# KentaYoshii/Raymarcher

Hardware: AMD Instinct MI355X
Metric: Mpixels/s at 3840x2160 Mandelbulb, 256 march steps (higher is better)
Workload: dtype f32

## Files before the change

### raymarcher_amd/csrc/rm_device.hip.h

```cpp
#pragma once
#include "../../include/raymarcher_amd.h"
#include <type_traits>

#include "rm_math.hip.h"
#include "rm_internal.h"

namespace rm {

struct V3 { float x, y, z; };
struct V4 { float x, y, z, w; };

RM_DEV V3 v3(float x, float y, float z) { return V3{x, y, z}; }
RM_DEV V4 v4(float x, float y, float z, float w) { return V4{x, y, z, w}; }
RM_DEV V3 add(V3 a, V3 b) { return v3(a.x + b.x, a.y + b.y, a.z + b.z); }
RM_DEV V3 sub(V3 a, V3 b) { return v3(a.x - b.x, a.y - b.y, a.z - b.z); }
RM_DEV V3 mul(V3 a, V3 b) { return v3(a.x * b.x, a.y * b.y, a.z * b.z); }
RM_DEV V3 scale(V3 a, float s) { return v3(a.x * s, a.y * s, a.z * s); }
RM_DEV V3 neg(V3 a) { return v3(-a.x, -a.y, -a.z); }
RM_DEV V3 madd(V3 a, float s, V3 b) { return v3(fma(a.x, s, b.x), fma(a.y, s, b.y), fma(a.z, s, b.z)); }
RM_DEV float dot2(float ax, float ay, float bx, float by) { return fma(ay, by, ax * bx); }
RM_DEV float dot(V3 a, V3 b) { return fma(a.z, b.z, fma(a.y, b.y, a.x * b.x)); }
RM_DEV float len2(float x, float y) { return sqrt_(dot2(x, y, x, y)); }
RM_DEV float len(V3 a) { return sqrt_(dot(a, a)); }
RM_DEV V3 normalize(V3 a) { float inv = rcp_(len(a)); return scale(a, inv); }
// ... 312 lines not shown
}
template <int COUNT>
RM_DEV SceneMin sdSceneOne(const SceneBlock *sb, int j, V3 p, Counters &cnt) {
  SceneMin res;
  res.trap = v4(0.0f, 0.0f, 0.0f, 0.0f);
  res.idx = j;
  if (COUNT) { cnt.evals++; cnt.shapes++; }
  const EvalRecord &o = sb->evalRec[j];
  float M[12];
#pragma unroll
  for (int c = 0; c < 12; c++) M[c] = o.m[c];
  const V3 po = v3(fma(M[6], p.z, fma(M[3], p.y, fma(M[0], p.x, M[9]))),
                   fma(M[7], p.z, fma(M[4], p.y, fma(M[1], p.x, M[10]))),
                   fma(M[8], p.z, fma(M[5], p.y, fma(M[2], p.x, M[11]))));
  float d = 0.0f;
  switch (o.type) {
    case RM_CUBE: d = sdBox(po, 0.5f, 0.5f, 0.5f); break;
    case RM_CONE: d = sdCone(po, 0.5f, 0.5f); break;
    case RM_CYLINDER: d = sdCylinder(po, 0.5f, 0.5f); break;
    case RM_SPHERE: d = len(po) - 0.5f; break;
    case RM_OCTAHEDRON: d = sdOctahedron(po, 0.5f); break;
    case RM_TORUS: d = sdTorus(po, 0.5f, 0.125f); break;
    case RM_CAPSULE: d = sdCapsule(po, 0.5f, 0.1f); break;
    case RM_DEATHSTAR: d = sdDeathStar(po, 0.5f, 0.35f, 0.5f); break;
    default: d = sdBox(po, 0.5f, 0.5f, 0.0f); break;
  }
  res.d = d * o.scaleFactor;
  return res;
}
RM_DEV float nextMinBound(float d, float lipLen, float depth) {
  const float ub = fma(fabs_(d), lipLen, d);
  return fma(fabs_(ub), 1.0e-4f, ub) + fma(depth, 1.0e-6f, 1.0e-5f);
}

template <int BULB, int COUNT, bool SKIP = false>
RM_DEV V3 getNormal(const SceneBlock *sb, V3 p, Counters &cnt, float ub = __builtin_inff()) {
  const float ex = (1.0f * 0.5773f) * 0.0005f, ey = (-1.0f * 0.5773f) * 0.0005f;
  float d[4];
#pragma unroll 1
  for (int k = 0; k < 4; k++) {
    float ox = (k == 0 || k == 3) ? ex : ey;
    float oy = (k >= 2) ? ex : ey;
    float oz = (k == 1 || k == 3) ? ex : ey;
    float v = sdScene<BULB, COUNT, false, SKIP>(sb, v3(p.x + ox, p.y + oy, p.z + oz), cnt, ub).d;
    d[0] = (k == 0) ? v : d[0];
    d[1] = (k == 1) ? v : d[1];
    d[2] = (k == 2) ? v : d[2];
    d[3] = (k == 3) ? v : d[3];
  }
  V3 n;
  n.x = fma(ex, d[3], fma(ey, d[2], fma(ey, d[1], ex * d[0])));
  n.y = fma(ex, d[3], fma(ex, d[2], fma(ey, d[1], ey * d[0])));
  n.z = fma(ex, d[3], fma(ey, d[2], fma(ex, d[1], ey * d[0])));
  return normalize(n);
}

RM_DEV float bulbCullEnd(const SceneBlock *sb, V3 ro, V3 rd, float end, bool &own) {
  own = false;
  const RmObject &o = sb->objs[0];
  const float jx = sb->g.juliaSeed[0], jy = sb->g.juliaSeed[1];
  const float seed2 = fma(jx, jx, jy * jy);
  const bool ok = (sb->g.power == 8.0f) && (o.scaleFactor >= 0.01f) && (seed2 <= 4.0f);
  if (!ok) return end;
  const bool tight = (o.scaleFactor >= 0.05f) && (seed2 <= 1.2996f);
  const float R2 = tight ? 1.3225f : 4.41f;
  const float *M = o.invModel;
  const V3 po = v3(fma(M[8], ro.z, fma(M[4], ro.y, fma(M[0], ro.x, M[12]))), fma(M[9], ro.z, fma(M[5], ro.y, fma(M[1], ro.x, M[13]))),
                   fma(M[10], ro.z, fma(M[6], ro.y, fma(M[2], ro.x, M[14]))));
  const V3 pd = v3(fma(M[8], rd.z, fma(M[4], rd.y, M[0] * rd.x)), fma(M[9], rd.z, fma(M[5], rd.y, M[1] * rd.x)),
                   fma(M[10], rd.z, fma(M[6], rd.y, M[2] * rd.x)));
  const float a = dot(pd, pd), b = dot(po, pd), c = dot(po, po) - R2;
  const float disc = fma(b, b, -(a * c));
  float tExit = (sqrt_fast_(max_(disc, 0.0f)) - b) / a;
  tExit = fma(tExit, 1.0001f, 1.0e-3f);
  if (c > 0.0f && (b >= 0.0f || disc < 0.0f)) tExit = -1.0f;
  if (!(a > 0.0f)) return end;
  own = (tExit <= end) && (c > 0.0f || tExit > 0.0f);
  return min_(end, tExit);
}
RM_DEV float bulbCullEnd(const SceneBlock *sb, V3 ro, V3 rd, float end) {
  bool own;
  return bulbCullEnd(sb, ro, rd, end, own);
}
struct BulbCull { bool ok; float R2; };
RM_DEV BulbCull bulbCullSetup(const SceneBlock *sb) {
  const RmObject &o = sb->objs[0];
  const float jx = sb->g.juliaSeed[0], jy = sb->g.juliaSeed[1];
  const float seed2 = fma(jx, jx, jy * jy);
  BulbCull cu;
  cu.ok = (sb->g.power == 8.0f) && (o.scaleFactor >= 0.01f) && (seed2 <= 4.0f);
  const bool tight = (o.scaleFactor >= 0.05f) && (seed2 <= 1.2996f);
  cu.R2 = tight ? 1.3225f : 4.41f;
  return cu;
}
template <bool PLAIN>
RM_DEV float bulbCullEndPrepared(const SceneBlock *sb, const BulbCull &cu, V3 ro, V3 pd, float a, float end, bool &own) {
  own = false;
  if (!cu.ok) return end;
  V3 po = ro;
  float pp = dot(ro, ro);
  if (!PLAIN || __ballot(!(pp < __builtin_inff())) != 0ull) {
    const float *M = sb->objs[0].invModel;
    po = v3(fma(M[8], ro.z, fma(M[4], ro.y, fma(M[0], ro.x, M[12]))), fma(M[9], ro.z, fma(M[5], ro.y, fma(M[1], ro.x, M[13]))),
            fma(M[10], ro.z, fma(M[6], ro.y, fma(M[2], ro.x, M[14]))));
    pp = dot(po, po);
  }
  const float b = dot(po, pd), c = pp - cu.R2;
  const float disc = fma(b, b, -(a * c));
  float tExit = (sqrt_fast_(max_(disc, 0.0f)) - b) / a;
  tExit = fma(tExit, 1.0001f, 1.0e-3f);
  if (c > 0.0f && (b >= 0.0f || disc < 0.0f)) tExit = -1.0f;
  if (!(a > 0.0f)) return end;
  own = (tExit <= end) && (c > 0.0f || tExit > 0.0f);
  return min_(end, tExit);
}
template <bool HARD = true>
RM_DEV float sceneCullEnd(const SceneBlock *sb, V3 ro, V3 rd, float end, float R2) {
  if (!sb->cullOk || !(R2 > 0.0f)) return end;
  const V3 po = v3(ro.x - sb->cullC[0], ro.y - sb->cullC[1], ro.z - sb->cullC[2]);
  const float a = dot(rd, rd), b = dot(po, rd), c = dot(po, po) - R2;
  const float disc = fma(b, b, -(a * c));
  float tExit = (sqrt_fast_(max_(disc, 0.0f)) - b) / a;
  tExit = fma(tExit, 1.0001f, 1.0e-3f);
  if (c > 0.0f && (b >= 0.0f || disc < 0.0f)) tExit = -1.0f;
  if (!(a > 0.0f)) return end;
  if (HARD && sb->cullBoxOk) {
    const float tx = ((rd.x >= 0.0f ? sb->cullHi[0] : sb->cullLo[0]) - ro.x) * __builtin_amdgcn_rcpf(rd.x);
    const float ty = ((rd.y >= 0.0f ? sb->cullHi[1] : sb->cullLo[1]) - ro.y) * __builtin_amdgcn_rcpf(rd.y);
    const float tz = ((rd.z >= 0.0f ? sb->cullHi[2] : sb->cullLo[2]) - ro.z) * __builtin_amdgcn_rcpf(rd.z);
    const float tb = min_(min_(tx, ty), tz);
    tExit = min_(tExit, fma(fabs_(tb), 1.0e-4f, tb) + 1.0e-3f);
  }
  return min_(end, tExit);
}
template <int BULB, int COUNT, bool SHADOW, bool CULL = false>
RM_DEV MarchRes march(const SceneBlock *sb, V3 ro, V3 rd, float end, float side, Counters &cnt, float ub0 = __builtin_inff()) {
  bool own = false;
  if (CULL && COUNT != 1) {
    const bool softRay = SHADOW && sb->s.enableSoftShadow != 0;
    if (BULB && !softRay) end = bulbCullEnd(sb, ro, rd, end, own);
    else if (softRay) end = sceneCullEnd<false>(sb, ro, rd, end, sb->cullR2Soft);
    else end = sceneCullEnd<true>(sb, ro, rd, end, sb->cullR2);
  }
  float depth = 0.0f;
  float pen = 1.0f;
  SceneMin c;
  c.d = 1000000.0f; c.idx = -1; c.trap = v4(0.0f, 0.0f, 0.0f, 0.0f);
  const int steps = sb->s.maxSteps;
  const bool soft = SHADOW && sb->s.enableSoftShadow != 0;
  constexpr bool SKIP = CULL && !BULB && COUNT != 1;
  const float lipLen = SKIP ? (sb->cullLip * len(rd)) * 1.0001f : 0.0f;
  float ub = ub0;
  float second = -__builtin_inff();
  if constexpr (BULB != 0 && CULL && COUNT != 1) {
    static_assert(!SKIP, "the bulb classes have no single-object fast path");
    auto bulbLoop = [&](auto preTag) __attribute__((always_inline)) {
      constexpr bool PRE = decltype(preTag)::value;
      for (int i = 0; i < steps; i++) {
        if (PRE && depth > end) break;
        c = sdSceneImpl<BULB, COUNT, !SHADOW, false, false>(sb, madd(rd, depth, ro), cnt, ub, second);
        if (fabs_(c.d) < kSurfaceDist || (!PRE && depth > end)) break;
        if (SHADOW) {
          if (soft) pen = min_(pen, divr_(8.0f * c.d, depth));
          depth = depth + fabs_(c.d);
        } else {
          depth = fma(c.d, side, depth);
        }
      }
    };
    if (__ballot(!own) == 0ull) bulbLoop(std::true_type{});
    else bulbLoop(std::false_type{});
  } else
  for (int i = 0; i < steps; i++) {
    const V3 p = madd(rd, depth, ro);
    bool one = false;
    int nearU = 0;
    if (SKIP) {
      nearU = __builtin_amdgcn_readfirstlane(c.idx);
      one = sb->cullOneOk && __ballot(!(c.idx == nearU && nearU >= 0 && second > ub)) == 0ull;
    }
    if (SKIP && one) c = sdSceneOne<COUNT>(sb, nearU, p, cnt);
    else c = sdSceneImpl<BULB, COUNT, !SHADOW, SKIP, SKIP>(sb, p, cnt, ub, second);
    if (fabs_(c.d) < kSurfaceDist || depth > end) break;
    if (SHADOW) {
      if (soft) pen = min_(pen, divr_(8.0f * c.d, depth));
      depth = depth + fabs_(c.d);
    } else {
      depth = fma(c.d, side, depth);
    }
    if (SKIP) {
      ub = nextMinBound(c.d, lipLen, depth);
      second = fma(fabs_(c.d), -(lipLen * 1.0001f), second) - fma(depth, 1.0e-6f, 1.0e-5f);
    }
  }
  MarchRes r;
  bool hit = fabs_(c.d) < kSurfaceDist;
  r.obj = hit ? c.idx : -1;
  r.trap = c.trap;
  if (SHADOW) r.d = pen;
  else r.d = hit ? (depth - c.d) : depth;
  return r;
}

RM_DEV float permute(float x) {
  const float y = fma(x, 34.0f, 1.0f) * x;
  return fma(-289.0f, floor_(RM_DIVC(y, 289.0f)), y);
}
RM_DEV float taylorInvSqrt(float r) { return fma(-0.85373472095314f, r, 1.79284291400159f); }
RM_DEV float fade(float t) { return ((t * t) * t) * fma(t, fma(t, 6.0f, -15.0f), 10.0f); }

RM_DEV void pgrad(float ixyz, float &gx, float &gy, float &gz) {
  float x = RM_DIVC(ixyz, 7.0f);
  float y = fract_(RM_DIVC(floor_(x), 7.0f)) - 0.5f;
  x = fract_(x);
  float z = (0.5f - fabs_(x)) - fabs_(y);
  float sz = step_(z, 0.0f);
  gx = fma(-sz, step_(0.0f, x) - 0.5f, x);
  gy = fma(-sz, step_(0.0f, y) - 0.5f, y);
  gz = z;
}
RM_DEV float pcorner(float ixyz, float fx, float fy, float fz) {
// ... 487 lines not shown
        }
      } else {
        fin = hit || depth > end;
        if (!fin) {
          depth = depth + fabs_(c.d);
          step++;
          fin = step >= maxSteps;
        }
      }
      if (fin) {
        if (hit) atomicOr(&hitw[own >> 1], 1u << (((own & 1) << 4) + cur));
        cur = -1;
      }
    }
    if (__ballot(cur >= 0) == 0ull && next >= n) break;
  }
  __builtin_amdgcn_wave_barrier();
  return (hitw[lane >> 1] >> ((lane & 1) << 4)) & 0xffffu;
}

#ifndef RM_X_PREP_PARTS
#define RM_X_PREP_PARTS 3
#endif
template <int BULB, int COUNT, bool SHARE, bool PREP>
RM_DEV RenderOut renderPooled(const SceneBlock *sb, const RmObject *objs, V3 ro, V3 rd, const MarchRes &res, Hit &info,
                              float maxT, V3 bg, Counters &cnt) {
  constexpr bool PREP_B = PREP && (RM_X_PREP_PARTS & 1) != 0, PREP_AC = PREP && (RM_X_PREP_PARTS & 2) != 0;
  const bool surf = res.obj != -1;
  const int nl = sb->numLights;
  V3 p = v3(0.0f, 0.0f, 0.0f), N = p, so = p;
  float ao = 1.0f, dStart = -1.0f;
  uint32_t pend = 0u, hits = 0u;
  if (surf) {
    if (COUNT) cnt.shades++;
    p = madd(rd, res.d, ro);
    N = getNormal<BULB, COUNT>(sb, p, cnt);
    if (sb->s.features & RM_FEAT_PERLIN_BUMP) N = SHARE ? bumpNormalShared(N, p) : bumpNormal(N, p);
    if (sb->s.enableAmbientOcclusion) ao = calcAO<BULB, COUNT>(sb, p, N, cnt);
    so = shadowOrigin(p, N);
    bool shared = f2u(so.x) != 0x80000000u && f2u(so.y) != 0x80000000u && f2u(so.z) != 0x80000000u;
    uint32_t need = 0u;
    for (int i = 0; i < nl; i++) {
      const RmLight &li = sb->lights[i];
      const V3 L = PREP_AC ? preparedL(sb, i) : normalize(v3(-li.dir[0], -li.dir[1], -li.dir[2]));
      shared = shared && (fabs_(L.x) + fabs_(L.y) + fabs_(L.z) <= 2.0f);
      if (!(dot(N, L) <= 0.005f)) need |= 1u << i;
    }
    const int maxSteps = sb->s.maxSteps;
    if (need != 0u && maxSteps > 0) {
      if (!shared) {
        pend = need;
      } else {
        const float d0 = fabs_(sdScene<BULB, COUNT, false>(sb, so, cnt).d);
        if (d0 < kSurfaceDist) hits = need;
        else if (maxSteps > 1) { pend = need; dStart = d0; }
      }
    }
  }
  const uint32_t hitMask = hits | shadowPool<BULB, COUNT, PREP_B>(sb, so, pend, dStart, maxT, cnt);
  RenderOut out;
  if (!surf) {
    out.col = bg;
    out.isEnv = 1;
    out.d = maxT;
    return out;
  }
  out.isEnv = 0;
  out.d = res.d;
  const RmObject &o = objs[0];
  Material mat;
  mat.amb = v3(o.cAmbient[0], o.cAmbient[1], o.cAmbient[2]);
  mat.dif = getDiffuse<false>(sb, o, p);
  mat.spec = v3(o.cSpecular[0], o.cSpecular[1], o.cSpecular[2]);
  mat.shininess = o.shininess;
  const float ka = sb->g.ka, ks = sb->g.ks;
  const V3 total = v3((mat.amb.x * ka) * ao, (mat.amb.y * ka) * ao, (mat.amb.z * ka) * ao);
  const V3 ph = hardLightSum<PREP_AC>(sb, mat, N, v3(0.0f, 0.0f, 0.0f), normalize(neg(rd)), maxT, ks, hitMask, total);
  const V3 c = bulbTrapColor(res.trap.y, res.trap.z, res.trap.w);
  out.col = v3(c.x * (ph.x * 8.0f), c.y * (ph.y * 8.0f), c.z * (ph.z * 8.0f));
  info.p = p; info.n = N; info.rd = rd; info.obj = res.obj;
  return out;
}

template <int BULB, int COUNT, bool TEX, bool CULLS, int SPLIT = 0, bool POOL = false, bool SHARE = false, bool PREP = false>
RM_DEV RenderOut render(const SceneBlock *sb, const RmObject *objs, V3 ro, V3 rd, Hit &info, float side, float maxT,
                        V3 bg, Counters &cnt, LightSplit split = LightSplit{-1, nullptr, 0}) {
  RenderOut out;
  info.obj = -1;
  MarchRes res;
  if (SPLIT == 2) {
    const float *q = split.slot + 2 * sb->numLights;
    res.obj = __float_as_int(q[0]); res.d = q[1]; res.trap = v4(q[2], q[3], q[4], q[5]);
  } else {
    res = march<BULB, COUNT, false, CULLS>(sb, ro, rd, maxT, side, cnt);
    if (SPLIT == 1 && split.part == 0) {
      float *q = split.slot + 2 * sb->numLights;
      q[0] = __int_as_float(res.obj); q[1] = res.d; q[2] = res.trap.x; q[3] = res.trap.y; q[4] = res.trap.z; q[5] = res.trap.w;
    }
  }
  if (POOL && hardDirectionalOnly(sb)) return renderPooled<BULB, COUNT, SHARE, PREP>(sb, objs, ro, rd, res, info, maxT, bg, cnt);
  if (res.obj == -1) {
    out.col = (TEX && sb->s.enableSkyBox) ? sampleCube(sb->skybox, rd) : bg;
    out.isEnv = 1;
    out.d = maxT;
    return out;
  }
  out.isEnv = 0;
  out.d = res.d;
  if (COUNT) cnt.shades++;
  V3 p = madd(rd, res.d, ro);
  constexpr bool SKIP = CULLS && !BULB && COUNT != 1;
  float ubP = __builtin_inff();
  if (SKIP) {
    const float lipLen = (sb->cullLip * len(rd)) * 1.0001f;
    ubP = fma(kSurfaceDist, lipLen, kSurfaceDist) * 1.001f + fma(fabs_(res.d), 1.0e-6f, 1.0e-5f);
  }
  V3 pn = getNormal<BULB, COUNT, SKIP>(sb, p, cnt, SKIP ? fma(0.0005f, sb->cullLip * 1.001f, ubP) : ubP);
  if (sb->s.features & RM_FEAT_PERLIN_BUMP) pn = bumpNormal(pn, p);
  const RmObject &o = objs[BULB ? 0 : res.obj];
  if (TEX && o.isEmissive) {
    out.col = v3(o.color[0], o.color[1], o.color[2]);
    return out;
  }
  Material mat;
  mat.amb = v3(o.cAmbient[0], o.cAmbient[1], o.cAmbient[2]);
  mat.dif = getDiffuse<TEX>(sb, o, p);
  mat.spec = v3(o.cSpecular[0], o.cSpecular[1], o.cSpecular[2]);
  mat.shininess = o.shininess;
  const int type = BULB ? (int)RM_MANDELBULB : o.type;
  V3 ph = getPhong<BULB, COUNT, TEX, CULLS, SPLIT>(sb, objs, mat, pn, p, rd, maxT, cnt, ubP, split);
  V3 col = ph;
  if (type == RM_MANDELBULB) {
    V3 c = bulbTrapColor(res.trap.y, res.trap.z, res.trap.w);
    col = v3(c.x * (ph.x * 8.0f), c.y * (ph.y * 8.0f), c.z * (ph.z * 8.0f));
  } else if (type == RM_MENGERSPONGE) {
    V3 c = v3(fma(0.5f, cos_(fma(2.0f, res.trap.z, 0.0f)), 0.5f), fma(0.5f, cos_(fma(2.0f, res.trap.z, 1.0f)), 0.5f),
              fma(0.5f, cos_(fma(2.0f, res.trap.z, 2.0f)), 0.5f));
    col = mul(c, ph);
  }
  info.p = p; info.n = pn; info.rd = rd; info.obj = res.obj;
  out.col = col;
  return out;
}

struct QuadCoord { float I, J; bool upper; };
RM_DEV QuadCoord quadCoord(int px, int py, int W, int H) {
  const float tx = ((float)px + 0.5f) / (float)W, ty = ((float)py + 0.5f) / (float)H;
  QuadCoord q;
  q.upper = (tx + ty) > 1.0f;
  q.I = q.upper ? 1.0f - tx : tx;
  q.J = q.upper ? 1.0f - ty : ty;
  return q;
}
RM_DEV void pixelNdc(int px, int py, int W, int H, float &ndcx, float &ndcy) {
  const QuadCoord q = quadCoord(px, py, W, H);
  ndcx = q.upper ? fma(q.I, -2.0f, 1.0f) : fma(q.I, 2.0f, -1.0f);
  ndcy = q.upper ? fma(q.J, -2.0f, 1.0f) : fma(q.J, 2.0f, -1.0f);
}
RM_DEV void primaryRay(const SceneBlock *sb, int px, int py, int W, int H, V3 &ro, V3 &rd) {
  const QuadCoord q = quadCoord(px, py, W, H);
  float nc[4], fc4[4];
#pragma unroll
  for (int k = 0; k < 4; k++) {
    const float (*A)[3][4] = sb->rayPlane[0], (*B)[3][4] = sb->rayPlane[1];
    auto sc = [](float v) { return u2f((uint32_t)__builtin_amdgcn_readfirstlane((int)f2u(v))); };
    const float p0n = q.upper ? sc(B[0][0][k]) : sc(A[0][0][k]), p1n = q.upper ? sc(B[0][1][k]) : sc(A[0][1][k]),
                p2n = q.upper ? sc(B[0][2][k]) : sc(A[0][2][k]);
    const float p0f = q.upper ? sc(B[1][0][k]) : sc(A[1][0][k]), p1f = q.upper ? sc(B[1][1][k]) : sc(A[1][1][k]),
                p2f = q.upper ? sc(B[1][2][k]) : sc(A[1][2][k]);
    nc[k] = fma(q.J, p2n, fma(q.I, p1n, p0n));
    fc4[k] = fma(q.J, p2f, fma(q.I, p1f, p0f));
  }
  ro = v3(nc[0] / nc[3], nc[1] / nc[3], nc[2] / nc[3]);
  V3 fc = v3(fc4[0] / fc4[3], fc4[1] / fc4[3], fc4[2] / fc4[3]);
  rd = normalize(sub(fc, ro));
}
RM_DEV V3 backgroundColor(const SceneBlock *sb) {
  V3 bg = v3(0.0f, 0.0f, 0.0f);
  if (sb->s.features & RM_FEAT_WHITE_BACKGROUND) bg = v3(1.0f, 1.0f, 1.0f);
  if (sb->s.features & RM_FEAT_DARK_BACKGROUND) bg = v3(0.0f, 0.0f, 0.0f);
  return bg;
}
RM_DEV V3 backgroundColor(const SceneBlock *sb, V3 rd) {
  V3 bg = v3(0.0f, 0.0f, 0.0f);
  if (sb->s.features & RM_FEAT_SKY_BACKGROUND) bg = getSky(rd);
  if (sb->s.features & RM_FEAT_NIGHTSKY_BACKGROUND) bg = getMoonColor(sb->noise, sb->g.iTime, rd);
  if (sb->s.features & RM_FEAT_WHITE_BACKGROUND) bg = v3(1.0f, 1.0f, 1.0f);
  if (sb->s.features & RM_FEAT_DARK_BACKGROUND) bg = v3(0.0f, 0.0f, 0.0f);
  return bg;
}

template <int BULB, int COUNT, bool ENV, bool TEX, bool SEC = true, int SPLIT = 0, bool RAY = false, bool SHARE = true,
          bool PREP = SHARE>
RM_DEV void shadePixel(const SceneBlock *sb, const RmObject *objs, int px, int py, int W, int H, V4 &fragColor,
                       V4 &bright, Counters &cnt, bool &hitFlag, LightSplit split = LightSplit{-1, nullptr, 0},
                       const V3 *rayO = nullptr, const V3 *rayD = nullptr) {
  float ndcx, ndcy;
  if (!RAY) pixelNdc(px, py, W, H, ndcx, ndcy);
  bright = v4(0.0f, 0.0f, 0.0f, 1.0f);
  hitFlag = false;
  if (!RAY && sb->g.isTwoD) {
    float s = sdMandelBrot(sb, ndcx, ndcy);
    fragColor = v4(pow_(s, 0.9f), pow_(s, 1.1f), pow_(s, 1.4f), 1.0f);
    return;
  }
  V3 ro, rd;
  if (RAY) { ro = *rayO; rd = *rayD; }
  else primaryRay(sb, px, py, W, H, ro, rd);
  const V3 bg = ENV ? backgroundColor(sb, rd) : backgroundColor(sb);
  const uint32_t feat = sb->s.features;
  const bool env = ENV && (feat & (RM_FEAT_TERRAIN | RM_FEAT_CLOUD | RM_FEAT_SEA)) != 0;
  const float far = (ENV && (feat & RM_FEAT_CLOUD)) ? 2000.0f : sb->cam.initialFar;
  const float iTime = sb->g.iTime;

  Hit info;
  constexpr bool POOL = BULB && !ENV && !TEX && COUNT != 1 && SPLIT == 0;
  RenderOut ri = render<BULB, COUNT, TEX, !ENV, SPLIT, POOL, SHARE, PREP>(sb, objs, ro, rd, info, 1.0f, far, bg, cnt, split);
  EnvOut e;
  e.terrainHit = false; e.cloudHit = false; e.seaHit = false;
  if (env) e = envLayers(feat, sb->noise, iTime, W, ro, rd, ri.d, bg, cnt);
  if (ri.isEnv && !e.cloudHit && !e.terrainHit && !e.seaHit) {
    fragColor = v4(ri.col.x, ri.col.y, ri.col.z, 1.0f);
    return;
  }
  if (e.cloudHit || e.terrainHit || e.seaHit) {
    V3 c = e.cloudHit ? e.ccol : (e.terrainHit ? e.tcol : e.scol);
    fragColor = v4(c.x, c.y, c.z, 1.0f);
    if (dot(c, v3(0.2126f, 0.7152f, 0.0722f)) > 1.0f) bright = v4(c.x, c.y, c.z, 1.0f);
    return;
  }
  hitFlag = true;
  V4 phong = v4(ri.col.x, ri.col.y, ri.col.z, 1.0f);
  V4 refl = v4(0.0f, 0.0f, 0.0f, 0.0f), refr = v4(0.0f, 0.0f, 0.0f, 0.0f);
  const Hit oi = info;
  const bool noObj = TEX && info.obj < 0;
  const RmObject &o = objs[(BULB || noObj) ? 0 : info.obj];
  const V3 cRefl = noObj ? v3(0.0f, 0.0f, 0.0f) : v3(o.cReflective[0], o.cReflective[1], o.cReflective[2]);
  const V3 cRefr = noObj ? v3(0.0f, 0.0f, 0.0f) : v3(o.cTransparent[0], o.cTransparent[1], o.cTransparent[2]);
  const float ior = o.ior;
  if (SEC && sb->s.enableReflection && len(cRefl) != 0.0f) {
    V3 fil = v3(1.0f, 1.0f, 1.0f);
    const int nb = sb->s.numReflection;
    for (int i = 0; i < nb; i++) {
      V3 r = reflect(info.rd, info.n);
      V3 sro = v3(fma(r.x * kSurfaceDist, 3.0f, info.p.x), fma(r.y * kSurfaceDist, 3.0f, info.p.y),
                  fma(r.z * kSurfaceDist, 3.0f, info.p.z));
      fil = mul(fil, cRefl);
      RenderOut res = render<BULB, COUNT, TEX, !ENV>(sb, objs, sro, r, info, 1.0f, far, bg, cnt);
      if (env) {
        EnvOut b = envLayers(feat, sb->noise, iTime, W, sro, r, res.d, bg, cnt);
        if (b.seaHit) res.col = b.scol;
        if (b.terrainHit) { res.col = b.tcol; res.isEnv = 1; }
        if (b.cloudHit) { res.col = b.ccol; res.isEnv = 1; }
      }
      refl.x += (sb->g.ks * fil.x) * res.col.x;
      refl.y += (sb->g.ks * fil.y) * res.col.y;
      refl.z += (sb->g.ks * fil.z) * res.col.z;
      refl.w += 1.0f;
      if (res.isEnv) break;
    }
  }
  if (SEC && sb->s.enableRefraction && len(cRefr) != 0.0f) {
    V3 rdIn = refract(oi.rd, oi.n, 1.0f / ior);
    V3 pEnter = v3(fma(-(oi.n.x * kSurfaceDist), 3.0f, oi.p.x), fma(-(oi.n.y * kSurfaceDist), 3.0f, oi.p.y),
                   fma(-(oi.n.z * kSurfaceDist), 3.0f, oi.p.z));
    float dIn = march<BULB, COUNT, false>(sb, pEnter, rdIn, far, -1.0f, cnt).d;
    V3 pExit = madd(rdIn, dIn, pEnter);
    V3 nExit = neg(getNormal<BULB, COUNT>(sb, pExit, cnt));
    V3 rdOut = refract(rdIn, nExit, ior);
    if (len(rdOut) != 0.0f) {
      V3 sro = v3(fma(-(nExit.x * kSurfaceDist), 5.0f, pExit.x), fma(-(nExit.y * kSurfaceDist), 5.0f, pExit.y),
                  fma(-(nExit.z * kSurfaceDist), 5.0f, pExit.z));
      RenderOut res = render<BULB, COUNT, TEX, !ENV>(sb, objs, sro, rdOut, info, 1.0f, far, bg, cnt);
      if (env) {
        EnvOut b = envLayers(feat, sb->noise, iTime, W, sro, rdOut, res.d, bg, cnt);
        if (b.seaHit) res.col = b.scol;
        if (b.terrainHit) res.col = b.tcol;
        if (b.cloudHit) res.col = b.ccol;
      }
      refr.x += (sb->g.kt * cRefr.x) * res.col.x;
      refr.y += (sb->g.kt * cRefr.y) * res.col.y;
      refr.z += (sb->g.kt * cRefr.z) * res.col.z;
      refr.w += 1.0f;
    }
  }
  fragColor = v4((phong.x + refl.x) + refr.x, (phong.y + refl.y) + refr.y, (phong.z + refl.z) + refr.z,
                 (phong.w + refl.w) + refr.w);
  V3 c = v3(fragColor.x, fragColor.y, fragColor.z);
  float brightness = dot(c, v3(0.2126f, 0.7152f, 0.0722f));
  if (brightness > 1.0f) bright = v4(c.x, c.y, c.z, 1.0f);
}
template <int BULB, int COUNT, bool ENV, bool TEX, bool SEC = true, int SPLIT = 0>
RM_DEV void shadeRay(const SceneBlock *sb, const RmObject *objs, V3 ro, V3 rd, int W, V4 &fragColor, V4 &bright, Counters &cnt,
                     bool &hitFlag, LightSplit split = LightSplit{-1, nullptr, 0}) {
  shadePixel<BULB, COUNT, ENV, TEX, SEC, SPLIT, true>(sb, objs, 0, 0, W, 1, fragColor, bright, cnt, hitFlag, split, &ro, &rd);
}

template <bool ENV, bool TEX>
RM_DEV void stageWorkgroup(const SceneBlock *sb, RmObject *s_objs) {
  const int nd = sb->numObjects * (int)(sizeof(RmObject) / 4);
// ... 14 lines not shown
```

### raymarcher_amd/csrc/rm_kernels.hip

```cpp
#include <hip/hip_runtime.h>

#include "rm_device.hip.h"
#include "rm_wavefront.hip.h"
#include "rm_internal.h"
#include "rm_frame.h"
#include "rm_launch.h"

namespace rm {

template <int BULB, int COUNT, bool ENV, bool TEX, bool SEC = true, int SPLIT = 0>
__global__ __launch_bounds__(256, render_waves(BULB, ENV, TEX, SEC)) void render_kernel(
    const SceneBlock *__restrict__ sb, RowMap map, int W, int H, int nRows, float4 *__restrict__ out, float4 *__restrict__ bright,
    unsigned long long *__restrict__ counters) {
  constexpr int CM = (COUNT == 3) ? 0 : COUNT;
  constexpr bool FRAMES = COUNT == 0 && SPLIT == 0;
  if (FRAMES) sb += blockIdx.z;
  unsigned long long t0 = 0, r0 = 0;
  if (COUNT == 3) { t0 = __builtin_amdgcn_s_memtime(); r0 = __builtin_amdgcn_s_memrealtime(); }
  __shared__ RmObject s_objs[BULB ? 1 : RM_MAX_OBJECTS];
  {
    const int nd = sb->numObjects * (int)(sizeof(RmObject) / 4);
    const uint32_t *src = reinterpret_cast<const uint32_t *>(sb->objs);
    uint32_t *dst = reinterpret_cast<uint32_t *>(s_objs);
    for (int i = threadIdx.x; i < nd; i += blockDim.x) dst[i] = src[i];
  }
  if (TEX || (ENV && (sb->s.features & (RM_FEAT_NIGHTSKY_BACKGROUND | RM_FEAT_SEA)))) initUnormTable();
  __syncthreads();
  const int wave = threadIdx.x >> 6, lane = threadIdx.x & 63;
  int tile = blockIdx.y * gridDim.x + blockIdx.x;
  const int32_t *order = sb->tileOrder;
  const int tsh = sb->tileShift, tw = 1 << tsh;
  int tilesX = (int)gridDim.x;
  LightSplit split{-1, nullptr, 0};
  if (SPLIT) {
    const int nl = sb->numLights, K = sb->splitTiles, b = (int)blockIdx.x;
    tilesX = (W + tw - 1) / tw;
    int h = b;
    if (SPLIT == 1) {
      if (b < K * nl) { h = b / nl; split.part = b - h * nl; }
      else h = K + (b - K * nl);
    }
    tile = order[h];
    if (h < K) {
      split.tileIndex = h;
      split.slot = sb->splitStore + (((size_t)K + 63) & ~(size_t)63) + ((size_t)h * 64 + lane) * (size_t)(2 * nl + 6);
    }
  } else if (order && sb->tileCount == (int)(gridDim.x * gridDim.y)) {
    tile = order[tile];
  }
  const int tbx = tile % tilesX, tby = tile / tilesX;
  __shared__ unsigned long long s_c0[4];
  if (!SPLIT && sb->tileCost && lane == 0) s_c0[wave] = __builtin_amdgcn_s_memtime();
  const int x = (tbx * (blockDim.x >> 6) + wave) * tw + (lane & (tw - 1));
  const int r = tby * (64 >> tsh) + (lane >> tsh);
  if (x >= W || r >= nRows) return;
  const int y = map.frameRow(r);
  V4 col, br;
  Counters cnt{0, 0, 0, 0, 0, 0};
  bool hit;
  shadePixel<BULB, CM, ENV, TEX, SEC, SPLIT>(sb, s_objs, x, y, W, H, col, br, cnt, hit, split);
  if (SPLIT == 1 && split.part >= 0) {
    __builtin_amdgcn_fence(__ATOMIC_RELEASE, "agent");
    uint32_t *arrived = reinterpret_cast<uint32_t *>(sb->splitStore) + split.tileIndex;
    const int leader = __builtin_ctzll(__ballot(1));
    uint32_t old = 0;
    if ((int)__lane_id() == leader) old = __hip_atomic_fetch_add(arrived, 1u, __ATOMIC_RELAXED, __HIP_MEMORY_SCOPE_AGENT);
    old = __shfl(old, leader);
    if ((int)old != sb->numLights - 1) return;
    __builtin_amdgcn_fence(__ATOMIC_ACQUIRE, "agent");
    split.part = -1;
    shadePixel<BULB, CM, ENV, TEX, SEC, 2>(sb, s_objs, x, y, W, H, col, br, cnt, hit, split);
  }
  if (FRAMES) {
    const size_t f = (size_t)sb->frame * (size_t)nRows * (size_t)W;
    out += f;
    if (bright) bright += f;
  }
  const size_t o = (size_t)r * W + x;
  out[o] = make_float4(col.x, col.y, col.z, col.w);
  if (bright) bright[o] = make_float4(br.x, br.y, br.z, br.w);
  if (CM) {
    atomicAdd(&counters[0], cnt.evals);
    atomicAdd(&counters[1], cnt.iters);
    if (hit) atomicAdd(&counters[2], 1ull);
    if (cnt.shades) atomicAdd(&counters[6], cnt.shades);
    if (cnt.fbm9) atomicAdd(&counters[7], cnt.fbm9);
    if (cnt.fbmd8) atomicAdd(&counters[8], cnt.fbmd8);
    if (cnt.shapes) atomicAdd(&counters[9], cnt.shapes);
  }
  if (!SPLIT && sb->tileCost && sb->tileCount == (int)(gridDim.x * gridDim.y)) {
    const unsigned long long c1 = __builtin_amdgcn_s_memtime();
    int t2 = blockIdx.y * gridDim.x + blockIdx.x;
    if (sb->tileOrder) t2 = sb->tileOrder[t2];
    if ((int)__lane_id() == __builtin_ctzll(__ballot(1))) atomicAdd(&sb->tileCost[t2], (uint32_t)((c1 - s_c0[wave]) >> 6));
  }
  if (COUNT == 3) {
    const unsigned long long t1 = __builtin_amdgcn_s_memtime(), r1 = __builtin_amdgcn_s_memrealtime();
    if ((int)__lane_id() == __builtin_ctzll(__ballot(1))) {
      atomicAdd(&counters[3], t1 - t0);
      atomicAdd(&counters[4], r1 - r0);
      unsigned long long *spans = reinterpret_cast<unsigned long long *>(counters[5]);
      if (spans) {
        int t3 = blockIdx.y * gridDim.x + blockIdx.x;
        if (sb->tileOrder && sb->tileCount == (int)(gridDim.x * gridDim.y)) t3 = sb->tileOrder[t3];
        const size_t w = (size_t)t3 * (blockDim.x >> 6) + wave;
        spans[2 * w] = r0;
        spans[2 * w + 1] = r1;
      }
    }
  }
}

RM_DEV void menger_uniforms(SceneBlock *sb) {
  sb->mengerAni = smoothstep_(-0.2f, 0.2f, -cos_(0.5f * sb->g.iTime));
  sb->mengerOff = 1.5f * sin_(0.01f * sb->g.iTime);
}
__global__ void scene_prep_batch_kernel(SceneBlock *sb, int n) {
  const int f = blockIdx.x * blockDim.x + threadIdx.x;
  if (f < n) menger_uniforms(sb + f);
}

constexpr int kOrderBuckets = 16;
RM_DEV int orderBucket(uint32_t cost) {
  const int lg = 31 - __builtin_clz(cost | 1u);
  const int b = 17 - lg;
  return b < 0 ? 0 : (b >= kOrderBuckets ? kOrderBuckets - 1 : b);
}
__global__ __launch_bounds__(256) void tile_hist_kernel(const uint32_t *__restrict__ cost, int n, uint32_t *__restrict__ hist) {
  __shared__ uint32_t s_cnt[kOrderBuckets];
  if (threadIdx.x < kOrderBuckets) s_cnt[threadIdx.x] = 0;
  __syncthreads();
  const int i = blockIdx.x * blockDim.x + threadIdx.x;
  const int b = i < n ? orderBucket(cost[i]) : -1;
  for (int k = 0; k < kOrderBuckets; k++) {
    const unsigned long long m = __ballot(b == k);
    if (m && (int)__lane_id() == __builtin_ctzll(m)) atomicAdd(&s_cnt[k], (uint32_t)__builtin_popcountll(m));
  }
  __syncthreads();
  if (threadIdx.x < kOrderBuckets && s_cnt[threadIdx.x]) atomicAdd(&hist[threadIdx.x], s_cnt[threadIdx.x]);
}
__global__ __launch_bounds__(256) void tile_scatter_kernel(uint32_t *__restrict__ cost, int n, uint32_t *__restrict__ hist,
                                                            int32_t *__restrict__ order, int keep) {
  __shared__ uint32_t s_cnt[kOrderBuckets], s_base[kOrderBuckets];
  if (threadIdx.x < kOrderBuckets) s_cnt[threadIdx.x] = 0;
  __syncthreads();
  const int i = blockIdx.x * blockDim.x + threadIdx.x;
  const int b = i < n ? orderBucket(cost[i]) : -1;
  uint32_t rank = 0;
  for (int k = 0; k < kOrderBuckets; k++) {
    const unsigned long long m = __ballot(b == k);
    if (!m) continue;
    uint32_t waveBase = 0;
    if ((int)__lane_id() == __builtin_ctzll(m)) waveBase = atomicAdd(&s_cnt[k], (uint32_t)__builtin_popcountll(m));
    waveBase = __shfl(waveBase, __builtin_ctzll(m));
    if (b == k) rank = waveBase + (uint32_t)__builtin_popcountll(m & ((1ull << __lane_id()) - 1ull));
  }
  __syncthreads();
  if (threadIdx.x < kOrderBuckets) {
    uint32_t start = 0;
    for (int k = 0; k < (int)threadIdx.x; k++) start += hist[k];
    s_base[threadIdx.x] = start + (s_cnt[threadIdx.x] ? atomicAdd(&hist[kOrderBuckets + threadIdx.x], s_cnt[threadIdx.x]) : 0u);
  }
  __syncthreads();
  if (i < n) {
    order[s_base[b] + rank] = i;
    if (!keep) cost[i] = 0u;
  }
}

__global__ __launch_bounds__(256) void tile_geom_kernel(const SceneBlock *__restrict__ sb, RowMap map, int W, int H, int nRows, int tilesX,
                                                        int tileW, int tileH, int n, const uint32_t *__restrict__ stale,
// ... 181 lines not shown
```

Measured before the change: 4808.

## Early-exit background waves in plain bulb kernel using primary ray cull

For the plain Mandelbulb kernel, each lane computes its primary ray and the bounding-sphere cull before shared-memory staging. If no lane in the wave can hit the bulb, the wave writes the background color and exits, skipping object staging when the block is a single wave. The precomputed ray and cull end are passed into march so they are not recomputed. This adds template variants and duplicated code, and it moves ray setup ahead of the barrier, which could raise register pressure.

```diff
diff --git a/raymarcher_amd/csrc/rm_device.hip.h b/raymarcher_amd/csrc/rm_device.hip.h
--- a/raymarcher_amd/csrc/rm_device.hip.h
+++ b/raymarcher_amd/csrc/rm_device.hip.h
@@ -418,6 +418,7 @@
   bool own;
   return bulbCullEnd(sb, ro, rd, end, own);
 }
+struct PrimaryCull { V3 ro, rd; float end; bool own; };
 struct BulbCull { bool ok; float R2; };
 RM_DEV BulbCull bulbCullSetup(const SceneBlock *sb) {
   const RmObject &o = sb->objs[0];
@@ -469,10 +470,14 @@
   }
   return min_(end, tExit);
 }
-template <int BULB, int COUNT, bool SHADOW, bool CULL = false>
-RM_DEV MarchRes march(const SceneBlock *sb, V3 ro, V3 rd, float end, float side, Counters &cnt, float ub0 = __builtin_inff()) {
+template <int BULB, int COUNT, bool SHADOW, bool CULL = false, bool GIVEN = false>
+RM_DEV MarchRes march(const SceneBlock *sb, V3 ro, V3 rd, float end, float side, Counters &cnt, float ub0 = __builtin_inff(),
+                      bool ownGiven = false) {
+  static_assert(!GIVEN || (BULB != 0 && CULL && COUNT != 1 && !SHADOW), "GIVEN: a hard primary ray of the culled bulb classes");
   bool own = false;
-  if (CULL && COUNT != 1) {
+  if (GIVEN) {
+    own = ownGiven;
+  } else if (CULL && COUNT != 1) {
     const bool softRay = SHADOW && sb->s.enableSoftShadow != 0;
     if (BULB && !softRay) end = bulbCullEnd(sb, ro, rd, end, own);
     else if (softRay) end = sceneCullEnd<false>(sb, ro, rd, end, sb->cullR2Soft);
@@ -1126,9 +1131,10 @@
   return out;
 }
 
-template <int BULB, int COUNT, bool TEX, bool CULLS, int SPLIT = 0, bool POOL = false, bool SHARE = false, bool PREP = false>
+template <int BULB, int COUNT, bool TEX, bool CULLS, int SPLIT = 0, bool POOL = false, bool SHARE = false, bool PREP = false,
+          bool GIVEN = false>
 RM_DEV RenderOut render(const SceneBlock *sb, const RmObject *objs, V3 ro, V3 rd, Hit &info, float side, float maxT,
-                        V3 bg, Counters &cnt, LightSplit split = LightSplit{-1, nullptr, 0}) {
+                        V3 bg, Counters &cnt, LightSplit split = LightSplit{-1, nullptr, 0}, const PrimaryCull *given = nullptr) {
   RenderOut out;
   info.obj = -1;
   MarchRes res;
@@ -1136,7 +1142,8 @@
     const float *q = split.slot + 2 * sb->numLights;
     res.obj = __float_as_int(q[0]); res.d = q[1]; res.trap = v4(q[2], q[3], q[4], q[5]);
   } else {
-    res = march<BULB, COUNT, false, CULLS>(sb, ro, rd, maxT, side, cnt);
+    if constexpr (GIVEN) res = march<BULB, COUNT, false, CULLS, true>(sb, ro, rd, given->end, side, cnt, __builtin_inff(), given->own);
+    else res = march<BULB, COUNT, false, CULLS>(sb, ro, rd, maxT, side, cnt);
     if (SPLIT == 1 && split.part == 0) {
       float *q = split.slot + 2 * sb->numLights;
       q[0] = __int_as_float(res.obj); q[1] = res.d; q[2] = res.trap.x; q[3] = res.trap.y; q[4] = res.trap.z; q[5] = res.trap.w;
@@ -1235,10 +1242,11 @@
 }
 
 template <int BULB, int COUNT, bool ENV, bool TEX, bool SEC = true, int SPLIT = 0, bool RAY = false, bool SHARE = true,
-          bool PREP = SHARE>
+          bool PREP = SHARE, bool GIVEN = false>
 RM_DEV void shadePixel(const SceneBlock *sb, const RmObject *objs, int px, int py, int W, int H, V4 &fragColor,
                        V4 &bright, Counters &cnt, bool &hitFlag, LightSplit split = LightSplit{-1, nullptr, 0},
-                       const V3 *rayO = nullptr, const V3 *rayD = nullptr) {
+                       const V3 *rayO = nullptr, const V3 *rayD = nullptr, const PrimaryCull *given = nullptr) {
+  static_assert(!GIVEN || (!RAY && !ENV), "GIVEN: a pixel's ray, far = sb->cam.initialFar");
   float ndcx, ndcy;
   if (!RAY) pixelNdc(px, py, W, H, ndcx, ndcy);
   bright = v4(0.0f, 0.0f, 0.0f, 1.0f);
@@ -1250,6 +1258,7 @@
   }
   V3 ro, rd;
   if (RAY) { ro = *rayO; rd = *rayD; }
+  else if (GIVEN) { ro = given->ro; rd = given->rd; }
   else primaryRay(sb, px, py, W, H, ro, rd);
   const V3 bg = ENV ? backgroundColor(sb, rd) : backgroundColor(sb);
   const uint32_t feat = sb->s.features;
@@ -1259,7 +1268,7 @@
 
   Hit info;
   constexpr bool POOL = BULB && !ENV && !TEX && COUNT != 1 && SPLIT == 0;
-  RenderOut ri = render<BULB, COUNT, TEX, !ENV, SPLIT, POOL, SHARE, PREP>(sb, objs, ro, rd, info, 1.0f, far, bg, cnt, split);
+  RenderOut ri = render<BULB, COUNT, TEX, !ENV, SPLIT, POOL, SHARE, PREP, GIVEN>(sb, objs, ro, rd, info, 1.0f, far, bg, cnt, split, given);
   EnvOut e;
   e.terrainHit = false; e.cloudHit = false; e.seaHit = false;
   if (env) e = envLayers(feat, sb->noise, iTime, W, ro, rd, ri.d, bg, cnt);
diff --git a/raymarcher_amd/csrc/rm_kernels.hip b/raymarcher_amd/csrc/rm_kernels.hip
--- a/raymarcher_amd/csrc/rm_kernels.hip
+++ b/raymarcher_amd/csrc/rm_kernels.hip
@@ -8,24 +8,40 @@
 
 namespace rm {
 
+#ifndef RM_X_BG_EXIT
+#define RM_X_BG_EXIT 1
+#endif
 template <int BULB, int COUNT, bool ENV, bool TEX, bool SEC = true, int SPLIT = 0>
 __global__ __launch_bounds__(256, render_waves(BULB, ENV, TEX, SEC)) void render_kernel(
     const SceneBlock *__restrict__ sb, RowMap map, int W, int H, int nRows, float4 *__restrict__ out, float4 *__restrict__ bright,
     unsigned long long *__restrict__ counters) {
   constexpr int CM = (COUNT == 3) ? 0 : COUNT;
   constexpr bool FRAMES = COUNT == 0 && SPLIT == 0;
+  constexpr bool BGX = RM_X_BG_EXIT != 0 && BULB == kBulbPlain && !ENV && !TEX && COUNT != 1 && SPLIT == 0;
   if (FRAMES) sb += blockIdx.z;
   unsigned long long t0 = 0, r0 = 0;
   if (COUNT == 3) { t0 = __builtin_amdgcn_s_memtime(); r0 = __builtin_amdgcn_s_memrealtime(); }
   __shared__ RmObject s_objs[BULB ? 1 : RM_MAX_OBJECTS];
-  {
-    const int nd = sb->numObjects * (int)(sizeof(RmObject) / 4);
-    const uint32_t *src = reinterpret_cast<const uint32_t *>(sb->objs);
-    uint32_t *dst = reinterpret_cast<uint32_t *>(s_objs);
-    for (int i = threadIdx.x; i < nd; i += blockDim.x) dst[i] = src[i];
-  }
-  if (TEX || (ENV && (sb->s.features & (RM_FEAT_NIGHTSKY_BACKGROUND | RM_FEAT_SEA)))) initUnormTable();
-  __syncthreads();
+  auto stage = [&]() __attribute__((always_inline)) {
+    {
+      const int nd = sb->numObjects * (int)(sizeof(RmObject) / 4);
+      const uint32_t *src = reinterpret_cast<const uint32_t *>(sb->objs);
+      uint32_t *dst = reinterpret_cast<uint32_t *>(s_objs);
+      for (int i = threadIdx.x; i < nd; i += blockDim.x) dst[i] = src[i];
+    }
+    if (TEX || (ENV && (sb->s.features & (RM_FEAT_NIGHTSKY_BACKGROUND | RM_FEAT_SEA)))) initUnormTable();
+    __syncthreads();
+  };
+  if constexpr (!BGX) {
+    {
+      const int nd = sb->numObjects * (int)(sizeof(RmObject) / 4);
+      const uint32_t *src = reinterpret_cast<const uint32_t *>(sb->objs);
+      uint32_t *dst = reinterpret_cast<uint32_t *>(s_objs);
+      for (int i = threadIdx.x; i < nd; i += blockDim.x) dst[i] = src[i];
+    }
+    if (TEX || (ENV && (sb->s.features & (RM_FEAT_NIGHTSKY_BACKGROUND | RM_FEAT_SEA)))) initUnormTable();
+    __syncthreads();
+  }
   const int wave = threadIdx.x >> 6, lane = threadIdx.x & 63;
   int tile = blockIdx.y * gridDim.x + blockIdx.x;
   const int32_t *order = sb->tileOrder;
@@ -53,12 +69,64 @@
   if (!SPLIT && sb->tileCost && lane == 0) s_c0[wave] = __builtin_amdgcn_s_memtime();
   const int x = (tbx * (blockDim.x >> 6) + wave) * tw + (lane & (tw - 1));
   const int r = tby * (64 >> tsh) + (lane >> tsh);
+  auto store = [&](V4 col, V4 br) __attribute__((always_inline)) {
+    if (FRAMES) {
+      const size_t f = (size_t)sb->frame * (size_t)nRows * (size_t)W;
+      out += f;
+      if (bright) bright += f;
+    }
+    const size_t o = (size_t)r * W + x;
+    out[o] = make_float4(col.x, col.y, col.z, col.w);
+    if (bright) bright[o] = make_float4(br.x, br.y, br.z, br.w);
+  };
+  auto stamps = [&]() __attribute__((always_inline)) {
+    if (!SPLIT && sb->tileCost && sb->tileCount == (int)(gridDim.x * gridDim.y)) {
+      const unsigned long long c1 = __builtin_amdgcn_s_memtime();
+      int t2 = blockIdx.y * gridDim.x + blockIdx.x;
+      if (sb->tileOrder) t2 = sb->tileOrder[t2];
+      if ((int)__lane_id() == __builtin_ctzll(__ballot(1))) atomicAdd(&sb->tileCost[t2], (uint32_t)((c1 - s_c0[wave]) >> 6));
+    }
+    if (COUNT == 3) {
+      const unsigned long long t1 = __builtin_amdgcn_s_memtime(), r1 = __builtin_amdgcn_s_memrealtime();
+      if ((int)__lane_id() == __builtin_ctzll(__ballot(1))) {
+        atomicAdd(&counters[3], t1 - t0);
+        atomicAdd(&counters[4], r1 - r0);
+        unsigned long long *spans = reinterpret_cast<unsigned long long *>(counters[5]);
+        if (spans) {
+          int t3 = blockIdx.y * gridDim.x + blockIdx.x;
+          if (sb->tileOrder && sb->tileCount == (int)(gridDim.x * gridDim.y)) t3 = sb->tileOrder[t3];
+          const size_t w = (size_t)t3 * (blockDim.x >> 6) + wave;
+          spans[2 * w] = r0;
+          spans[2 * w + 1] = r1;
+        }
+      }
+    }
+  };
+  PrimaryCull pc;
+  if constexpr (BGX) {
+    const bool inFrame = x < W && r < nRows;
+    bool bgWave = false;
+    if (sb->g.isTwoD == 0) {
+      primaryRay(sb, x, map.frameRow(r), W, H, pc.ro, pc.rd);
+      pc.end = bulbCullEnd(sb, pc.ro, pc.rd, sb->cam.initialFar, pc.own);
+      bgWave = __ballot(inFrame && !(pc.own && pc.end < 0.0f)) == 0ull;
+    }
+    if (!(bgWave && blockDim.x == 64)) stage();
+    if (bgWave) {
+      if (!inFrame) return;
+      const V3 bg = backgroundColor(sb);
+      store(v4(bg.x, bg.y, bg.z, 1.0f), v4(0.0f, 0.0f, 0.0f, 1.0f));
+      stamps();
+      return;
+    }
+  }
   if (x >= W || r >= nRows) return;
   const int y = map.frameRow(r);
   V4 col, br;
   Counters cnt{0, 0, 0, 0, 0, 0};
   bool hit;
-  shadePixel<BULB, CM, ENV, TEX, SEC, SPLIT>(sb, s_objs, x, y, W, H, col, br, cnt, hit, split);
+  if constexpr (BGX) shadePixel<BULB, CM, ENV, TEX, SEC, SPLIT, false, true, true, true>(sb, s_objs, x, y, W, H, col, br, cnt, hit, split, nullptr, nullptr, &pc);
+  else shadePixel<BULB, CM, ENV, TEX, SEC, SPLIT>(sb, s_objs, x, y, W, H, col, br, cnt, hit, split);
   if (SPLIT == 1 && split.part >= 0) {
     __builtin_amdgcn_fence(__ATOMIC_RELEASE, "agent");
     uint32_t *arrived = reinterpret_cast<uint32_t *>(sb->splitStore) + split.tileIndex;
@@ -71,14 +139,18 @@
     split.part = -1;
     shadePixel<BULB, CM, ENV, TEX, SEC, 2>(sb, s_objs, x, y, W, H, col, br, cnt, hit, split);
   }
-  if (FRAMES) {
-    const size_t f = (size_t)sb->frame * (size_t)nRows * (size_t)W;
-    out += f;
-    if (bright) bright += f;
-  }
-  const size_t o = (size_t)r * W + x;
-  out[o] = make_float4(col.x, col.y, col.z, col.w);
-  if (bright) bright[o] = make_float4(br.x, br.y, br.z, br.w);
+  if constexpr (BGX) {
+    store(col, br);
+  } else {
+    if (FRAMES) {
+      const size_t f = (size_t)sb->frame * (size_t)nRows * (size_t)W;
+      out += f;
+      if (bright) bright += f;
+    }
+    const size_t o = (size_t)r * W + x;
+    out[o] = make_float4(col.x, col.y, col.z, col.w);
+    if (bright) bright[o] = make_float4(br.x, br.y, br.z, br.w);
+  }
   if (CM) {
     atomicAdd(&counters[0], cnt.evals);
     atomicAdd(&counters[1], cnt.iters);
@@ -87,6 +159,10 @@
     if (cnt.fbm9) atomicAdd(&counters[7], cnt.fbm9);
     if (cnt.fbmd8) atomicAdd(&counters[8], cnt.fbmd8);
     if (cnt.shapes) atomicAdd(&counters[9], cnt.shapes);
+  }
+  if constexpr (BGX) {
+    stamps();
+    return;
   }
   if (!SPLIT && sb->tileCost && sb->tileCount == (int)(gridDim.x * gridDim.y)) {
     const unsigned long long c1 = __builtin_amdgcn_s_memtime();
```

Result: no change. 4834, median of 6 (+0.6%).
